# samuelkriegerbonini-dev/AstroBurst

Hardware: AMD Instinct MI355X
Metric: MPix/s sigma-clipped stack+stretch, 64x4096x4096 f32 (higher is better)
Workload: dtype f32

## Files before the change

### astroburst_amd/csrc/tile_stream.hpp

```cpp
#pragma once
#include <hip/hip_runtime.h>

#include <cstdint>

#include "ab_common.hpp"
#include "tile_bucket.hpp"

namespace ts {

using tb::dev_key;
using tb::wave_scan_incl;
using tb::wave_sort64;
using tb::Window;

constexpr int kThreads = 256;
constexpr int kWaves = kThreads / 64;
constexpr int kBuckets = 4096;
constexpr int kTop = kBuckets - 1;
constexpr int kPer = kBuckets / kThreads;
constexpr int kHotCap = 3072;
constexpr int kTabCap = 384;
constexpr int kSelCap = 1024;
constexpr int kMaxZones = 16;
constexpr int kRing = 2;
constexpr int kRingPlan = 3;
constexpr int kEdgePlan = 12;
#ifndef TS_PER_SIGMA
#define TS_PER_SIGMA 480.0f
#endif
constexpr float kPerSigma = TS_PER_SIGMA;
constexpr unsigned int kNone = 0xffffffffu;

enum Decline {
    D_NONE = 0, D_ZONES, D_HOT_OVERFLOW, D_MED_CATCHALL, D_MED_COLD, D_MED_BIG, D_DEV_BM, D_DEV_NOFIRST, D_DEV_SHAPE, D_DEV_COLD,
    D_DEV_BIG, D_DEV_COUNT, D_DEV_PROOF, D_EDGE_COLD, D_EDGE_CATCHALL, D_SAMPLE
};

struct alignas(16) Shared {
    unsigned int prefix[kBuckets + kThreads];
    float list[kHotCap + kThreads];
    union {
        unsigned char lut[kBuckets];
        unsigned int tmp[kSelCap];
    };
    unsigned int zcur[kMaxZones + kThreads];
    uint32_t tab_first[kTabCap], tab_last[kTabCap];
    unsigned int part[4 * kWaves];
    unsigned int zone_at[kMaxZones + 1];
    int zone_lo[kMaxZones], zone_hi[kMaxZones];
    int zone_tab[kMaxZones];
    int nzones;
    int decline;
    unsigned int ncand;
#ifdef AB_TILE_TIMING
    long long t_phase[16];
    long long t_mark;
#endif
};

#ifdef AB_TILE_TIMING
#define TS_MARK(sh, i)                             \
    do {                                           \
        if (threadIdx.x == 0) {                    \
            const long long now_ = clock64();      \
            (sh).t_phase[i] += now_ - (sh).t_mark; \
            (sh).t_mark = now_;                    \
        }                                          \
    } while (0)
#else
#define TS_MARK(sh, i) \
    do {               \
    } while (0)
#endif

__device__ __forceinline__ uint32_t ord_of(float x) {
    const uint32_t b = __float_as_uint(x);
    return b ^ ((b >> 31) ? 0xffffffffu : 0x80000000u);
}
__device__ __forceinline__ float from_ord(uint32_t u) { return __uint_as_float(u ^ ((u >> 31) ? 0x80000000u : 0xffffffffu)); }

struct Geo {
    float scale, off;
    float r_min, r_max;
    ab_pixel_xf xf;
    double range;
    __device__ __forceinline__ int bucket(float v) const { return (int)__builtin_amdgcn_fmed3f(__builtin_fmaf(v, scale, off), 0.0f, (float)kTop); }
    __device__ __forceinline__ bool is_cand(float v) const { return v >= r_min && v <= r_max; }
    __device__ __forceinline__ uint32_t norm_key(float raw) const { return __float_as_uint(ab_px(xf, raw)); }
    __device__ __forceinline__ float unnorm(float x) const { return xf.on ? (float)((double)x * range + xf.lo) : x; }
    __device__ __forceinline__ int bucket_at_norm(float x) const { return bucket(unnorm(x)); }
    __device__ __forceinline__ bool first_raw(int b, float *out) const {
        uint32_t u = ord_of(((float)b - off) / scale);
        int guard = 0;
        while (bucket(from_ord(u)) >= b && ++guard < 64) --u;
        while (bucket(from_ord(u)) < b && ++guard < 128) ++u;
        *out = from_ord(u);
        return guard < 128 && bucket(from_ord(u)) >= b && bucket(from_ord(u - 1u)) < b;
    }
    __device__ __forceinline__ bool first_norm(int b, uint32_t *key) const {
        if (b <= 0) {
            *key = 0x33d6bf96u;
            return true;
        }
        float r;
        if (!first_raw(b, &r)) return false;
        *key = norm_key(r < r_min ? r_min : r);
        return true;
    }
    __device__ __forceinline__ bool last_norm(int b, uint32_t *key) const {
        if (b >= kTop) {
            *key = norm_key(r_max);
            return true;
        }
        float r;
        if (!first_raw(b + 1, &r)) return false;
        r = from_ord(ord_of(r) - 1u);
        *key = norm_key(r < r_min ? r_min : r);
        return true;
    }
};

__device__ __forceinline__ void scan_prefix(Shared &sh) {
    const int t = threadIdx.x, b0 = t * kPer, w = t >> 6, lane = t & 63;
    unsigned int v[kPer];
#pragma unroll
    for (int j = 0; j < kPer; j += 4) {
        const uint4 q = *reinterpret_cast<const uint4 *>(&sh.prefix[b0 + j]);
        v[j] = q.x;
        v[j + 1] = q.y;
        v[j + 2] = q.z;
        v[j + 3] = q.w;
    }
#pragma unroll
    for (int j = 1; j < kPer; ++j) v[j] += v[j - 1];
    const unsigned int tot = v[kPer - 1], incl = wave_scan_incl(tot);
    if (lane == 63) sh.part[w] = incl;
    __syncthreads();
    unsigned int before = incl - tot;
#pragma unroll
    for (int i = 0; i < kWaves; ++i) before += i < w ? sh.part[i] : 0u;
#pragma unroll
    for (int j = 0; j < kPer; j += 4) {
        uint4 q;
        q.x = v[j] + before;
        q.y = v[j + 1] + before;
        q.z = v[j + 2] + before;
        q.w = v[j + 3] + before;
        *reinterpret_cast<uint4 *>(&sh.prefix[b0 + j]) = q;
    }
    __syncthreads();
}

__device__ __forceinline__ void wave_sync() { __builtin_amdgcn_fence(__ATOMIC_ACQ_REL, "wavefront"); }
__device__ __forceinline__ int first_lane(unsigned long long m) { return (int)__builtin_ctzll(m); }
__device__ __forceinline__ unsigned int lanes_below(unsigned long long m) {
    return __builtin_amdgcn_mbcnt_hi((unsigned int)(m >> 32), __builtin_amdgcn_mbcnt_lo((unsigned int)m, 0u));
}
__device__ __forceinline__ unsigned int below(const Shared &sh, int b) { return b <= 0 ? 0u : sh.prefix[b - 1]; }

__device__ __forceinline__ int wfind_rank(const Shared &sh, unsigned int g) {
    const int lane = threadIdx.x & 63;
    const unsigned long long m1 = __builtin_amdgcn_ballot_w64(g < sh.prefix[64 * lane + 63]);
    const int L = m1 ? first_lane(m1) : 63;
    const unsigned long long m2 = __builtin_amdgcn_ballot_w64(g < sh.prefix[64 * L + lane]);
    return 64 * L + (m2 ? first_lane(m2) : 63);
}

__device__ __forceinline__ unsigned int wprefix(const Shared &sh, const Window &w, int b) {
    const unsigned int p = below(sh, b);
    const unsigned int q = p < w.c_lo ? w.c_lo : (p > w.c_le_hi ? w.c_le_hi : p);
    return q - w.c_lo;
}

struct ZReg {
    int lo, hi, tab;
    unsigned int at, end;
    int n;
    __device__ __forceinline__ void load(const Shared &sh) {
        const int lane = threadIdx.x & 63;
        n = sh.nzones;
        const bool have = lane < n;
        lo = have ? sh.zone_lo[lane] : 0;
        hi = have ? sh.zone_hi[lane] : -1;
        tab = have ? sh.zone_tab[lane] : -1;
        at = have ? sh.zone_at[lane] : 0u;
        end = have ? sh.zone_at[lane + 1] : 0u;
    }
    __device__ __forceinline__ int zone_of(int b) const {
        const unsigned long long m = __builtin_amdgcn_ballot_w64(b >= lo && b <= hi);
        return m ? first_lane(m) : -1;
    }
    __device__ __forceinline__ int lo_of(int z) const { return __builtin_amdgcn_readlane(lo, z); }
    __device__ __forceinline__ int hi_of(int z) const { return __builtin_amdgcn_readlane(hi, z); }
    __device__ __forceinline__ unsigned int at_of(int z) const { return (unsigned int)__builtin_amdgcn_readlane((int)at, z); }
    __device__ __forceinline__ unsigned int end_of(int z) const { return (unsigned int)__builtin_amdgcn_readlane((int)end, z); }
    __device__ __forceinline__ int tab_index(int b) const {
        const unsigned long long m = __builtin_amdgcn_ballot_w64(tab >= 0 && b >= lo - 1 && b <= hi + 1);
        if (!m) return -1;
        const int z = first_lane(m);
        return __builtin_amdgcn_readlane(tab, z) + (b - __builtin_amdgcn_readlane(lo, z) + 1);
    }
};
__device__ __forceinline__ bool tfirst(const Shared &sh, const ZReg &zr, const Geo &g, int b, uint32_t *key) {
    const int i = zr.tab_index(b);
    if (i < 0) return g.first_norm(b, key);
    *key = sh.tab_first[i];
    return *key != 0u;
}
__device__ __forceinline__ bool tlast(const Shared &sh, const ZReg &zr, const Geo &g, int b, uint32_t *key) {
    const int i = zr.tab_index(b);
    if (i < 0) return g.last_norm(b, key);
    *key = sh.tab_last[i];
    return *key != 0u;
}

struct DevGeo {
    float mf;
    float delta;
    int bm;
};
__device__ __forceinline__ void ring_of(const Geo &g, const DevGeo &d, float t, int *bl, int *br) {
    const int l = g.bucket_at_norm(d.mf - t), r = g.bucket_at_norm(d.mf + t);
    *bl = l < d.bm ? l : d.bm;
    *br = r > d.bm ? r : d.bm;
}
__device__ __forceinline__ bool make_devgeo(const Shared &sh, const ZReg &zr, const Geo &g, double median, DevGeo *d) {
    d->mf = (float)median;
    int b = g.bucket_at_norm(d->mf), guard = 0;
    uint32_t k;
    auto first_le = [&](int bb, bool *le) {
        if (!tfirst(sh, zr, g, bb, &k)) return false;
        *le = (double)__uint_as_float(k) <= median;
        return true;
    };
    bool le;
    while (b > 0) {
        if (!first_le(b, &le)) return false;
        if (le || ++guard > 8) break;
        --b;
    }
    while (b < kTop) {
        if (!first_le(b + 1, &le)) return false;
        if (!le || ++guard > 16) break;
        ++b;
    }
    d->bm = b;
    if (b <= 0 || b >= kTop || guard > 16) return false;
    uint32_t k0, k1;
    if (!tfirst(sh, zr, g, b, &k0) || !tfirst(sh, zr, g, b + 1, &k1)) return false;
    d->delta = __uint_as_float(k1) - __uint_as_float(k0);
    return d->delta > 0.0f;
}

__device__ __forceinline__ unsigned int wmad_first(const Shared &sh, const Geo &g, const Window &w, const DevGeo &d, unsigned int need, unsigned int guess) {
    const int lane = threadIdx.x & 63;
    auto reaches = [&](unsigned int i) {
        int bl, br;
        ring_of(g, d, (float)(i + 1u) * d.delta, &bl, &br);
        return wprefix(sh, w, br + 1) - wprefix(sh, w, bl) >= need;
    };
    if (guess != kNone) {
        const unsigned int gi = guess < 3900u ? guess : 3900u, i_lo = gi > 96u ? gi - 96u : 0u;
#pragma unroll 1
        for (int j = 0; j < 4; ++j) {
            const unsigned long long m = __builtin_amdgcn_ballot_w64(reaches(i_lo + 64u * j + lane));
            if (m) {
                const unsigned int first = i_lo + 64u * j + (unsigned int)first_lane(m);
                if (first > i_lo || i_lo == 0u) return first;
                break;
            }
        }
    }
#pragma unroll 1
    for (int j = 0; j < kBuckets / 64; ++j) {
        const unsigned long long m = __builtin_amdgcn_ballot_w64(reaches(64u * j + lane));
        if (m) return 64u * j + (unsigned int)first_lane(m);
    }
    return kNone;
}

__device__ __forceinline__ int plan_zones(Shared &sh, const Geo &g, unsigned int cnt, float mad_guess, unsigned int (&first_guess)[3]) {
    int nz = 0;
    auto add = [&](int lo, int hi) {
        lo = lo < 1 ? 1 : lo;
        hi = hi > kTop - 1 ? kTop - 1 : hi;
        if (lo <= hi && nz < kMaxZones) {
            if ((threadIdx.x & 63) == 0) {
                sh.zone_lo[nz] = lo;
                sh.zone_hi[nz] = hi;
            }
            ++nz;
        }
    };
    Window w;
    w.lo = 1;
    w.hi = 0x7f7fffffu;
    w.c_lo = 0;
    w.c_le_hi = cnt;
    w.n = cnt;
    first_guess[0] = first_guess[1] = first_guess[2] = kNone;
#pragma unroll 1
    for (int it = 0; it < 3; ++it) {
        if (w.n < 3) break;
        const unsigned int mid = w.n / 2, g_hi = w.c_lo + mid, g_lo = w.n % 2 == 0 ? g_hi - 1 : g_hi;
        const int b_hi = wfind_rank(sh, g_hi), b_lo = g_lo == g_hi ? b_hi : wfind_rank(sh, g_lo);
        add(b_lo - 1, b_hi + 1);
        if (b_hi <= 0 || b_hi >= kTop) break;
        uint32_t k0, k1;
        if (!g.first_norm(b_hi, &k0) || !g.first_norm(b_hi + 1, &k1)) break;
        const unsigned int ex = below(sh, b_hi), in_b = sh.prefix[b_hi] - ex;
        const float frac = ((float)(g_hi - ex) + 0.5f) / (float)(in_b ? in_b : 1u);
        const float v0 = __uint_as_float(k0), v1 = __uint_as_float(k1);
        const double med = (double)(v0 + frac * (v1 - v0));
        DevGeo d;
        d.mf = (float)med;
        d.bm = b_hi;
        d.delta = v1 - v0;
        if (!(d.delta > 0.0f)) break;
        unsigned int guess = kNone;
        if (it == 0) {
            if (mad_guess > 0.0f) {
                const float gi = mad_guess / d.delta;
                guess = gi < 3900.0f ? (unsigned int)gi : 3900u;
            }
        } else {
            guess = first_guess[it - 1];
        }
        const unsigned int first = wmad_first(sh, g, w, d, mid + 1u, guess);
        if (first == kNone) break;
        first_guess[it] = first;
        {
            int bLo, bRo, bLi = d.bm, bRi = d.bm;
            ring_of(g, d, (float)(first + 1u + kRing + kRingPlan) * d.delta, &bLo, &bRo);
            if (first + 1u > (unsigned int)(kRing + kRingPlan)) ring_of(g, d, (float)(first + 1u - kRing - kRingPlan) * d.delta, &bLi, &bRi);
            if (bLi + 1 >= bRi) {
                add(bLo, bRo);
            } else {
                add(bLo, bLi);
                add(bRi, bRo);
            }
        }
        if (it == 2) break;
        const double mad = (double)(((float)first + 0.5f) * d.delta);
        const double sig = fmax(mad * 1.4826, 1e-30);
        const float lo = (float)(med - 3.0 * sig), hi = (float)(med + 3.0 * sig);
        if (!(lo <= hi)) break;
        const float e = (float)kEdgePlan * d.delta;
        int bl = 0, bh = kTop;
        if (lo > 0.0f) {
            add(g.bucket_at_norm(lo - e), g.bucket_at_norm(lo + e));
            bl = g.bucket_at_norm(lo);
        }
        if (hi < 3.0e38f) {
            add(g.bucket_at_norm(hi - e), g.bucket_at_norm(hi + e));
            bh = g.bucket_at_norm(hi);
        }
        unsigned int c_lo = lo > 0.0f ? below(sh, bl) + (sh.prefix[bl] - below(sh, bl)) / 2u : 0u;
        unsigned int c_hi = hi < 3.0e38f ? sh.prefix[bh] - (sh.prefix[bh] - below(sh, bh)) / 2u : cnt;
        c_lo = c_lo > w.c_lo ? c_lo : w.c_lo;
        c_hi = c_hi < w.c_le_hi ? c_hi : w.c_le_hi;
        if (c_hi <= c_lo) break;
        w.c_lo = c_lo;
        w.c_le_hi = c_hi;
        w.n = c_hi - c_lo;
    }
    return nz;
}

__device__ __forceinline__ bool build_zones(Shared &sh, const Geo &g, int nz) {
    const int lane = threadIdx.x & 63;
    wave_sync();
    uint32_t key = lane < nz ? ((uint32_t)sh.zone_lo[lane] << 16) | (uint32_t)sh.zone_hi[lane] : kNone;
    key = wave_sort64(key);
    int m = 0, cur_lo = 0, cur_hi = -2;
    int my_lo = 0, my_hi = -1;
    for (int i = 0; i < nz; ++i) {
        const uint32_t k = (uint32_t)__builtin_amdgcn_readlane((int)key, i);
        const int lo = (int)(k >> 16), hi = (int)(k & 0xffffu);
        if (m > 0 && lo <= cur_hi + 1) {
            cur_hi = hi > cur_hi ? hi : cur_hi;
        } else {
            if (m > 0 && lane == m - 1) {
                my_lo = cur_lo;
                my_hi = cur_hi;
            }
            cur_lo = lo;
            cur_hi = hi;
            ++m;
        }
    }
    if (m > 0 && lane == m - 1) {
        my_lo = cur_lo;
        my_hi = cur_hi;
    }
    const unsigned int size = lane < m ? sh.prefix[my_hi] - below(sh, my_lo) : 0u;
    const unsigned int tlen = lane < m ? (unsigned int)(my_hi - my_lo + 3) : 0u;
    const unsigned int at = wave_scan_incl(size) - size, tat = wave_scan_incl(tlen) - tlen;
    if (lane < m) {
        sh.zone_lo[lane] = my_lo;
        sh.zone_hi[lane] = my_hi;
        sh.zone_at[lane] = at;
        sh.zcur[lane] = at;
        sh.zone_tab[lane] = tat + tlen <= (unsigned int)kTabCap ? (int)tat : -1;
        if (lane == m - 1) sh.zone_at[m] = at + size;
    }
    if (lane == 0) sh.nzones = m;
    wave_sync();
    return m != 0 && sh.zone_at[m] <= (unsigned int)kHotCap;
}
__device__ __forceinline__ void fill_zone_tables(Shared &sh, const Geo &g) {
    const int t = threadIdx.x, m = sh.nzones;
    for (int z = 0; z < m; ++z) {
        const int lo = sh.zone_lo[z], hi = sh.zone_hi[z], tb0 = sh.zone_tab[z];
        for (int b = lo + t; b <= hi; b += kThreads) sh.lut[b] = (unsigned char)(z + 1);
        if (tb0 >= 0)
            for (int b = lo - 1 + t; b <= hi + 1; b += kThreads) {
                uint32_t kf = 0u, kl = 0u;
                if (!g.first_norm(b, &kf)) kf = 0u;
                if (!g.last_norm(b, &kl)) kl = 0u;
                sh.tab_first[tb0 + (b - lo + 1)] = kf;
                sh.tab_last[tb0 + (b - lo + 1)] = kl;
            }
    }
}

__device__ __forceinline__ void wselect2(Shared &sh, unsigned int n, unsigned int r_lo, unsigned int r_hi, uint32_t *k_lo, uint32_t *k_hi) {
    constexpr int kMine = kSelCap / 64;
    const int lane = threadIdx.x & 63;
    unsigned int *const hist = &sh.prefix[kBuckets];
    wave_sync();
    if (n <= 64u) {
        const uint32_t sorted = wave_sort64((unsigned int)lane < n ? sh.tmp[lane] : kNone);
        *k_lo = (uint32_t)__builtin_amdgcn_readlane((int)sorted, (int)r_lo);
        *k_hi = (uint32_t)__builtin_amdgcn_readlane((int)sorted, (int)r_hi);
        return;
    }
    uint32_t mine[kMine];
    const uint32_t k0 = sh.tmp[0];
    uint32_t diff = 0;
#pragma unroll
    for (int q = 0; q < kMine; ++q) {
        const unsigned int i = (unsigned int)(q * 64 + lane);
        mine[q] = i < n ? sh.tmp[i] : k0;
        diff |= mine[q] ^ k0;
    }
#pragma unroll
    for (int off = 32; off >= 1; off >>= 1) diff |= (uint32_t)__shfl_xor((int)diff, off, 64);
    int top = 24;
    while (top > 0 && (diff >> top) == 0) top -= 8;
    uint32_t mask = top == 24 ? 0u : (0xffffffffu << (top + 8));
    uint32_t prefix = k0 & mask;
    unsigned int rank = r_hi;
    for (int shift = top; shift >= 0; shift -= 8) {
        *reinterpret_cast<uint4 *>(&hist[4 * lane]) = make_uint4(0u, 0u, 0u, 0u);
        wave_sync();
#pragma unroll
        for (int q = 0; q < kMine; ++q)
            if ((unsigned int)(q * 64) < n) {
                if ((unsigned int)(q * 64 + lane) < n && (mine[q] & mask) == prefix) atomicAdd(&hist[(mine[q] >> shift) & 255u], 1u);
            }
        wave_sync();
        const uint4 c = *reinterpret_cast<const uint4 *>(&hist[4 * lane]);
        const unsigned int own = c.x + c.y + c.z + c.w;
        const unsigned int incl = wave_scan_incl(own);
        const unsigned int excl = incl - own;
        const bool owner = rank >= excl && rank < incl;
        uint32_t digit = 0;
        unsigned int bel = 0;
        if (owner) {
            const unsigned int r = rank - excl;
            if (r < c.x) {
                digit = 4 * lane;
                bel = excl;
            } else if (r < c.x + c.y) {
                digit = 4 * lane + 1;
                bel = excl + c.x;
            } else if (r < c.x + c.y + c.z) {
                digit = 4 * lane + 2;
                bel = excl + c.x + c.y;
            } else {
                digit = 4 * lane + 3;
                bel = excl + c.x + c.y + c.z;
            }
        }
        const unsigned long long om = __builtin_amdgcn_ballot_w64(owner);
        const int ol = om ? first_lane(om) : 0;
        digit = (uint32_t)__builtin_amdgcn_readlane((int)digit, ol);
        bel = (unsigned int)__builtin_amdgcn_readlane((int)bel, ol);
        rank -= bel;
        prefix |= digit << shift;
        mask |= 255u << shift;
    }
    *k_hi = prefix;
    *k_lo = prefix;
    if (r_lo != r_hi && rank == 0) {
        uint32_t best = 0;
#pragma unroll
        for (int q = 0; q < kMine; ++q)
            if ((unsigned int)(q * 64 + lane) < n && mine[q] < prefix) best = best > mine[q] ? best : mine[q];
        *k_lo = tb::wave_max(best);
    }
}

template <class KeyOf>
__device__ __forceinline__ unsigned int gather_keys(Shared &sh, unsigned int from, unsigned int to, uint32_t k_from, uint32_t k_to, unsigned int at,
                                                    KeyOf key_of) {
    const int lane = threadIdx.x & 63;
    const uint32_t *const list = reinterpret_cast<const uint32_t *>(sh.list);
#pragma unroll 1
    for (unsigned int i0 = from; i0 < to; i0 += 256) {
        uint32_t key[4];
#pragma unroll
        for (int j = 0; j < 4; ++j) {
            const unsigned int i = i0 + 64u * j + lane;
            const uint32_t k = i < to ? list[i] : 0u;
            key[j] = (k >= k_from && k <= k_to) ? key_of(k) : kNone;
        }
#pragma unroll
        for (int j = 0; j < 4; ++j) {
            const unsigned long long m = __builtin_amdgcn_ballot_w64(key[j] != kNone);
            const unsigned int pos = at + lanes_below(m);
            if (key[j] != kNone && pos < (unsigned int)kSelCap) sh.tmp[pos] = key[j];
            at += (unsigned int)__builtin_popcountll(m);
        }
        if (at > (unsigned int)kSelCap) return kNone;
    }
    return at;
}

struct Rounds {
    Shared &sh;
    const Geo &g;
    ZReg zr;
    __device__ __forceinline__ bool fail(int why) {
        sh.decline = why;
        return false;
    }
    __device__ __forceinline__ bool key_range(int ba, int bb, uint32_t *k_from, uint32_t *k_to) {
        uint32_t prev, next;
        if (!tfirst(sh, zr, g, ba, k_from) || !tlast(sh, zr, g, bb, k_to) || !tlast(sh, zr, g, ba - 1, &prev) || !tfirst(sh, zr, g, bb + 1, &next)) return false;
        if (prev >= *k_from && sh.prefix[ba - 1] != below(sh, ba - 1)) return false;
        if (next <= *k_to && sh.prefix[bb + 1] != sh.prefix[bb]) return false;
        return true;
    }
    __device__ __forceinline__ bool select_values(unsigned int g_lo, unsigned int g_hi, uint32_t *k_lo, uint32_t *k_hi) {
        const int b_hi = wfind_rank(sh, g_hi), b_lo = g_lo == g_hi ? b_hi : wfind_rank(sh, g_lo);
        if (b_lo <= 0 || b_hi >= kTop) return fail(D_MED_CATCHALL);
        const int z_lo = zr.zone_of(b_lo), z_hi = zr.zone_of(b_hi);
        if (z_lo < 0 || z_hi < 0) return fail(D_MED_COLD);
        auto same = [](uint32_t k) { return k; };
        uint32_t kf, kt;
        if (!key_range(b_lo, b_lo, &kf, &kt)) return fail(D_MED_COLD);
        unsigned int n = gather_keys(sh, zr.at_of(z_lo), zr.end_of(z_lo), kf, kt, 0u, same);
        if (n != kNone && b_hi != b_lo) {
            if (!key_range(b_hi, b_hi, &kf, &kt)) return fail(D_MED_COLD);
            n = gather_keys(sh, zr.at_of(z_hi), zr.end_of(z_hi), kf, kt, n, same);
        }
        if (n == kNone) return fail(D_MED_BIG);
        const unsigned int ex = below(sh, b_lo);
        if (n != sh.prefix[b_hi] - ex) return fail(D_MED_COLD);
        TS_MARK(sh, 8);
        wselect2(sh, n, g_lo - ex, g_hi - ex, k_lo, k_hi);
        TS_MARK(sh, 9);
        return true;
    }
    __device__ __forceinline__ bool select_devs(const Window &w, double median, unsigned int r_lo, unsigned int r_hi, unsigned int guess, uint32_t *d_lo,
                                                uint32_t *d_hi) {
        DevGeo d;
        if (!make_devgeo(sh, zr, g, median, &d)) return fail(D_DEV_BM);
        TS_MARK(sh, 10);
        const unsigned int first = wmad_first(sh, g, w, d, r_hi + 1u, guess);
        TS_MARK(sh, 11);
        if (first == kNone) return fail(D_DEV_NOFIRST);
        int bLo, bRo, bLi = 0, bRi = 0;
        ring_of(g, d, (float)(first + 1u + kRing) * d.delta, &bLo, &bRo);
        const bool has_inner_t = first + 1u > (unsigned int)kRing;
        if (has_inner_t) ring_of(g, d, (float)(first + 1u - kRing) * d.delta, &bLi, &bRi);
        const bool has_inner = has_inner_t && bLi + 1 <= bRi - 1;
        const unsigned int c_in = has_inner ? wprefix(sh, w, bRi) - wprefix(sh, w, bLi + 1) : 0u;
        const unsigned int n_cand = wprefix(sh, w, bRo + 1) - wprefix(sh, w, bLo) - c_in;
        if (!(bLo > 0 && bRo < kTop && c_in <= r_lo && c_in + n_cand >= r_hi + 1u && n_cand <= (unsigned int)kSelCap)) return fail(D_DEV_SHAPE);
        auto key_of = [&](uint32_t k) { return (k >= w.lo && k <= w.hi) ? dev_key(k, median) : kNone; };
        unsigned int n;
        uint32_t kf, kt;
        if (has_inner) {
            const int zl = zr.zone_of(bLo), zq = zr.zone_of(bRi);
            if (zl < 0 || zq < 0 || bLi > zr.hi_of(zl) || bRo > zr.hi_of(zq)) return fail(D_DEV_COLD);
            if (!key_range(bLo, bLi, &kf, &kt)) return fail(D_DEV_COLD);
            n = gather_keys(sh, zr.at_of(zl), zr.end_of(zl), kf, kt, 0u, key_of);
            if (n != kNone) {
                if (!key_range(bRi, bRo, &kf, &kt)) return fail(D_DEV_COLD);
                n = gather_keys(sh, zr.at_of(zq), zr.end_of(zq), kf, kt, n, key_of);
            }
        } else {
            const int z = zr.zone_of(bLo);
            if (z < 0 || bRo > zr.hi_of(z)) return fail(D_DEV_COLD);
            if (!key_range(bLo, bRo, &kf, &kt)) return fail(D_DEV_COLD);
            n = gather_keys(sh, zr.at_of(z), zr.end_of(z), kf, kt, 0u, key_of);
        }
        if (n == kNone) return fail(D_DEV_BIG);
        if (n != n_cand) return fail(D_DEV_COUNT);
        TS_MARK(sh, 12);
        uint32_t sel_lo, sel_hi;
        wselect2(sh, n, r_lo - c_in, r_hi - c_in, &sel_lo, &sel_hi);
        TS_MARK(sh, 13);
        uint32_t t_in = 0, t_out = kNone;
        if (has_inner) {
            uint32_t ka, kb;
            if (!tfirst(sh, zr, g, bLi + 1, &ka) || !tlast(sh, zr, g, bRi - 1, &kb)) return fail(D_DEV_PROOF);
            ka = ka > w.lo ? ka : w.lo;
            kb = kb < w.hi ? kb : w.hi;
            if (ka <= kb) {
                const uint32_t da = dev_key(ka, median), db = dev_key(kb, median);
                t_in = da > db ? da : db;
            }
        }
        if (wprefix(sh, w, bLo) > 0u) {
            uint32_t k;
            if (!tlast(sh, zr, g, bLo - 1, &k) || !((double)__uint_as_float(k) <= median)) return fail(D_DEV_PROOF);
            t_out = dev_key(k, median);
        }
        if (wprefix(sh, w, kBuckets) - wprefix(sh, w, bRo + 1) > 0u) {
            uint32_t k;
            if (!tfirst(sh, zr, g, bRo + 1, &k) || !((double)__uint_as_float(k) >= median)) return fail(D_DEV_PROOF);
            const uint32_t dd = dev_key(k, median);
            t_out = t_out < dd ? t_out : dd;
        }
        TS_MARK(sh, 14);
        if (!(t_in <= sel_lo && sel_hi <= t_out)) return fail(D_DEV_PROOF);
        *d_lo = sel_lo;
        *d_hi = sel_hi;
        return true;
    }
    template <bool HI>
    __device__ __forceinline__ bool count_edge(uint32_t bound, unsigned int *out) {
        const int lane = threadIdx.x & 63;
        int b = g.bucket_at_norm(__uint_as_float(bound)), guard = 0;
        auto reaches = [&](int bb, bool *r) {
            uint32_t k;
            if (!tlast(sh, zr, g, bb, &k)) return false;
            *r = HI ? k > bound : k >= bound;
            return true;
        };
        bool r;
        while (b > 0) {
            if (!reaches(b - 1, &r)) return fail(D_EDGE_COLD);
            if (!r || ++guard > 8) break;
            --b;
        }
        while (b < kTop) {
            if (!reaches(b, &r)) return fail(D_EDGE_COLD);
            if (r || ++guard > 16) break;
            ++b;
        }
        if (guard > 16) return fail(D_EDGE_COLD);
        const unsigned int bel = below(sh, b), in_b = sh.prefix[b] - bel;
        if (in_b == 0) {
            *out = bel;
            return true;
        }
        if (b <= 0 || b >= kTop) {
            uint32_t kf, kl;
            if (!tfirst(sh, zr, g, b, &kf) || !tlast(sh, zr, g, b, &kl)) return fail(D_EDGE_CATCHALL);
            if (HI ? kl <= bound : kl < bound) {
                *out = bel + in_b;
                return true;
            }
            if (HI ? kf > bound : kf >= bound) {
                *out = bel;
                return true;
            }
            return fail(D_EDGE_CATCHALL);
        }
        const int z = zr.zone_of(b);
        uint32_t kf, kt;
        if (z < 0 || !key_range(b, b, &kf, &kt)) return fail(D_EDGE_COLD);
        const uint32_t *const list = reinterpret_cast<const uint32_t *>(sh.list);
        unsigned int c = 0, seen = 0;
        const unsigned int to = zr.end_of(z);
        for (unsigned int i0 = zr.at_of(z); i0 < to; i0 += 256) {
#pragma unroll
            for (int j = 0; j < 4; ++j) {
                const unsigned int i = i0 + 64u * j + lane;
                const uint32_t k = i < to ? list[i] : 0u;
                const bool mine = k >= kf && k <= kt;
                seen += mine ? 1u : 0u;
                c += (mine && (HI ? k <= bound : k < bound)) ? 1u : 0u;
            }
        }
        seen = tb::wave_sum(seen);
        c = tb::wave_sum(c);
        if (seen != in_b) return fail(D_EDGE_COLD);
        *out = bel + c;
        return true;
    }

    __device__ __forceinline__ bool run(unsigned int cnt, const unsigned int (&first_guess)[3], double *median_out, double *sigma_out) {
        constexpr double kMadToSigma = 1.4826;
        zr.load(sh);
        Window w;
        w.lo = 1;
        w.hi = 0x7f7fffffu;
        w.c_lo = 0;
        w.c_le_hi = cnt;
        w.n = cnt;
        double median = 0.0, sigma = 1.0;
#pragma unroll 1
        for (int it = 0; it < 3; ++it) {
            if (it < 2 && w.n < 3) continue;
            if (w.n == 0) {
                median = 0.0;
                sigma = 1.0;
                break;
            }
            const unsigned int mid = w.n / 2;
            uint32_t ka, kb;
            if (!select_values(w.c_lo + (w.n % 2 == 0 ? mid - 1 : mid), w.c_lo + mid, &ka, &kb)) return false;
            median = w.n % 2 == 0 ? ((double)__uint_as_float(ka) + (double)__uint_as_float(kb)) / 2.0 : (double)__uint_as_float(kb);
            uint32_t da, db;
            if (!select_devs(w, median, w.n % 2 == 0 ? mid - 1 : mid, mid, first_guess[it], &da, &db)) return false;
            const float mad_f32 = w.n % 2 == 0 ? (__uint_as_float(da) + __uint_as_float(db)) / 2.0f : __uint_as_float(db);
            const double sig = fmax((double)mad_f32 * kMadToSigma, 1e-30);
            if (it == 2) {
                sigma = sig;
                break;
            }
            const float lo = (float)(median - 3.0 * sig), hi = (float)(median + 3.0 * sig);
            if (!(lo <= hi)) {
                w.n = 0;
                w.c_lo = w.c_le_hi = 0;
                w.lo = 1;
                w.hi = 0;
                continue;
            }
            const uint32_t klo = lo > 0.0f ? __float_as_uint(lo) : 1u;
            const uint32_t khi = hi > 0.0f ? (__float_as_uint(hi) > 0x7f7fffffu ? 0x7f7fffffu : __float_as_uint(hi)) : 0u;
            const bool new_lo = klo > w.lo, new_hi = khi < w.hi;
            w.lo = new_lo ? klo : w.lo;
            w.hi = new_hi ? khi : w.hi;
            if (w.lo > w.hi) {
                w.n = 0;
                w.c_lo = w.c_le_hi = 0;
                continue;
            }
            TS_MARK(sh, 6);
            if (new_lo && w.lo > 0x33d6bf96u && !count_edge<false>(w.lo, &w.c_lo)) return false;
            if (new_hi && !count_edge<true>(w.hi, &w.c_le_hi)) return false;
            w.n = w.c_le_hi - w.c_lo;
            TS_MARK(sh, 15);
        }
        *median_out = median;
        *sigma_out = sigma;
        return true;
    }
};

struct TileRect {
    const float *img;
    int64_t ld;
    int y0, y1, x0, x1;
    bool vec;
};
struct __attribute__((packed, aligned(4))) F4u {
    float x, y, z, w;
};
__device__ __forceinline__ float4 load4u(const float *p) {
    const F4u t = *reinterpret_cast<const F4u *>(p);
    return make_float4(t.x, t.y, t.z, t.w);
}
__device__ __forceinline__ bool whole_tile(const TileRect &r) { return r.vec && r.y1 - r.y0 == 256 && r.x1 - r.x0 == 256; }
template <class F>
__device__ __forceinline__ void stream_whole_tile_batches(const TileRect &r, F f) {
    constexpr int U = 4, kRounds = 64 / (2 * U);
    const int t = threadIdx.x, lane = t & 63, wv = t >> 6;
    const float *p = r.img + (int64_t)(r.y0 + wv) * r.ld + r.x0 + 4 * lane;
    const int64_t step = (int64_t)kWaves * r.ld;
    float4 A[U], B[U];
    auto load = [&](float4(&X)[U]) {
#pragma unroll
        for (int u = 0; u < U; ++u) X[u] = load4u(p + u * step);
        p += U * step;
    };
    unsigned int at = (unsigned int)(wv * 256 + 4 * lane);
    auto eat = [&](const float4(&X)[U]) {
        float v[4 * U];
#pragma unroll
        for (int u = 0; u < U; ++u) {
            v[4 * u + 0] = X[u].x;
            v[4 * u + 1] = X[u].y;
            v[4 * u + 2] = X[u].z;
            v[4 * u + 3] = X[u].w;
        }
        f(v, at);
        at += (unsigned int)(U * kWaves * 256);
    };
    load(A);
#pragma unroll 1
    for (int it = 0; it < kRounds; ++it) {
        load(B);
        eat(A);
        if (it + 1 < kRounds) load(A);
        eat(B);
    }
}
template <class F>
__device__ __forceinline__ void stream_tile(const TileRect &r, F f) {
    const int t = threadIdx.x;
    if (whole_tile(r)) {
        constexpr int U = 4, kRounds = 64 / (2 * U);
        const int lane = t & 63, wv = t >> 6;
        const float *p = r.img + (int64_t)(r.y0 + wv) * r.ld + r.x0 + 4 * lane;
        const int64_t step = (int64_t)kWaves * r.ld;
        float4 A[U], B[U];
        auto load = [&](float4(&X)[U]) {
#pragma unroll
            for (int u = 0; u < U; ++u) X[u] = load4u(p + u * step);
            p += U * step;
        };
        auto eat = [&](const float4(&X)[U]) {
#pragma unroll
            for (int u = 0; u < U; ++u) {
                f(X[u].x);
                f(X[u].y);
                f(X[u].z);
                f(X[u].w);
            }
        };
        load(A);
#pragma unroll 1
        for (int it = 0; it < kRounds; ++it) {
            load(B);
            eat(A);
            if (it + 1 < kRounds) load(A);
            eat(B);
        }
    } else if (r.vec) {
        constexpr int U = 8;
        const int lane = t & 63, wv = t >> 6, c = r.x0 + 4 * lane;
        const bool col_ok = c < r.x1;
        const float *p = r.img + c;
#pragma unroll 1
        for (int r0 = r.y0 + wv; r0 < r.y1; r0 += kWaves * U) {
            float4 raw[U];
#pragma unroll
            for (int u = 0; u < U; ++u) {
                const int row = r0 + kWaves * u;
                raw[u] = (col_ok && row < r.y1) ? load4u(p + (int64_t)row * r.ld)
                                                : make_float4(__builtin_nanf(""), __builtin_nanf(""), __builtin_nanf(""), __builtin_nanf(""));
            }
#pragma unroll
            for (int u = 0; u < U; ++u) {
                f(raw[u].x);
                f(raw[u].y);
                f(raw[u].z);
                f(raw[u].w);
            }
        }
    } else {
        constexpr int U = 16;
        const int c = r.x0 + t;
        const bool col_ok = c < r.x1;
        const float *p = r.img + c;
#pragma unroll 1
        for (int r0 = r.y0; r0 < r.y1; r0 += U) {
            float raw[U];
#pragma unroll
            for (int u = 0; u < U; ++u) raw[u] = (col_ok && r0 + u < r.y1) ? p[(int64_t)(r0 + u) * r.ld] : __builtin_nanf("");
#pragma unroll
            for (int u = 0; u < U; ++u) f(raw[u]);
        }
    }
}

struct TileResult {
    double median, sigma;
    int valid;
    int declined;
};

__device__ __forceinline__ void candidate_range(const ab_pixel_xf &xf, float *r_min, float *r_max) {
    if (!xf.on) {
        *r_min = __uint_as_float(0x33d6bf96u);
        *r_max = 3.4028234663852886e38f;
        return;
    }
    *r_max = __builtin_inff();
    uint32_t lo = ord_of(-__builtin_inff()), hi = ord_of(__builtin_inff());
    while (hi - lo > 1u) {
        const uint32_t mid = lo + ((hi - lo) >> 1);
        if (ab_px(xf, from_ord(mid)) > 1e-7f)
            hi = mid;
        else
            lo = mid;
    }
    *r_min = from_ord(hi);
}

__device__ __forceinline__ bool zoom_from_sample(Shared &sh, const TileRect &r, const ab_pixel_xf &xf, Geo *g, float *mad_guess) {
    const int t = threadIdx.x, lane = t & 63, wv = t >> 6;
    const int h = r.y1 - r.y0, wd = r.x1 - r.x0;
    g->xf = xf;
    g->range = xf.on ? 1.0 / xf.inv : 1.0;
    candidate_range(xf, &g->r_min, &g->r_max);
    const int sr = r.y0 + (int)(((unsigned int)t * (unsigned int)h) >> 8), sc = r.x0 + (int)(((unsigned int)(t * 67 + 13) % 256u * (unsigned int)wd) >> 8);
    const float sv = r.img[(int64_t)sr * r.ld + sc];
    const uint32_t sorted = wave_sort64(g->is_cand(sv) ? ord_of(sv) : 0u);
    const int nz = __builtin_popcountll(__builtin_amdgcn_ballot_w64(sorted == 0u)), nv = 64 - nz;
    const uint32_t q1 = (uint32_t)__shfl((int)sorted, nz + nv / 4 < 64 ? nz + nv / 4 : 63, 64);
    const uint32_t q2 = (uint32_t)__shfl((int)sorted, nz + nv / 2 < 64 ? nz + nv / 2 : 63, 64);
    const uint32_t q3 = (uint32_t)__shfl((int)sorted, nz + (3 * nv) / 4 < 64 ? nz + (3 * nv) / 4 : 63, 64);
    if (lane == 0) {
        sh.part[4 * wv + 0] = q1;
        sh.part[4 * wv + 1] = q2;
        sh.part[4 * wv + 2] = q3;
        sh.part[4 * wv + 3] = nv >= 8 ? 1u : 0u;
    }
    __syncthreads();
    float s1 = 0.0f, s2 = 0.0f, s3 = 0.0f, sn = 0.0f;
#pragma unroll
    for (int i = 0; i < kWaves; ++i) {
        const bool ok = sh.part[4 * i + 3] != 0u;
        s1 += ok ? from_ord(sh.part[4 * i + 0]) : 0.0f;
        s2 += ok ? from_ord(sh.part[4 * i + 1]) : 0.0f;
        s3 += ok ? from_ord(sh.part[4 * i + 2]) : 0.0f;
        sn += ok ? 1.0f : 0.0f;
    }
    __syncthreads();
    if (!(sn > 0.0f)) return false;
    const float Q1 = s1 / sn, Q2 = s2 / sn, Q3 = s3 / sn;
    const float sig = (Q3 - Q1) * (1.0f / 1.349f);
    const float wb = sig / kPerSigma;
    g->scale = 1.0f / wb;
    const float vlo = Q2 - (float)((kBuckets - 2) / 2) * wb;
    g->off = 1.0f - vlo * g->scale;
    *mad_guess = 0.6745f * sig * (float)(xf.on ? xf.inv : 1.0);
    return sig > 0.0f && __builtin_isfinite(g->scale) && __builtin_isfinite(g->off) && g->scale > 0.0f;
}

struct CandSink {
    uint2 *ent = nullptr;
    unsigned int *cnt = nullptr;
    float *cut = nullptr;
    unsigned int cap = 0;
};
#ifndef TS_CAND_SIGMAS
#define TS_CAND_SIGMAS 2.5f
#endif
constexpr float kCandSigmas = TS_CAND_SIGMAS;

__device__ __forceinline__ int rounds_wave() {
#ifdef TS_ROUNDS_WAVE0
    return 0;
#else
    return (int)(blockIdx.x & 3u);
#endif
}

__device__ __forceinline__ TileResult tile_stats(Shared &sh, const TileRect &r, const ab_pixel_xf &xf, const CandSink cs = CandSink()) {
    const int t = threadIdx.x;
    TileResult res = {0.0, 1.0, 0, 0};
    if (cs.cut && t == 0) {
        *cs.cut = __builtin_nanf("");
        *cs.cnt = 0u;
    }
#ifdef AB_TILE_TIMING
    if (t == 0) {
        for (int i = 0; i < 16; ++i) sh.t_phase[i] = 0;
        sh.t_mark = clock64();
    }
#endif
    if (t == 0) {
        sh.decline = D_NONE;
        sh.nzones = 0;
        sh.ncand = 0u;
    }
#pragma unroll
    for (int i = 0; i < kPer; i += 4) *reinterpret_cast<uint4 *>(&sh.prefix[t * kPer + i]) = make_uint4(0u, 0u, 0u, 0u);
    *reinterpret_cast<uint4 *>(&sh.lut[16 * t]) = make_uint4(0u, 0u, 0u, 0u);
    Geo g;
    float mad_guess;
    if (!zoom_from_sample(sh, r, xf, &g, &mad_guess)) {
        res.declined = D_SAMPLE;
        return res;
    }
    TS_MARK(sh, 0);
    stream_tile(r, [&](float v) { atomicAdd(&sh.prefix[g.is_cand(v) ? g.bucket(v) : kBuckets + t], 1u); });
    __syncthreads();
    TS_MARK(sh, 1);
    scan_prefix(sh);
    const unsigned int cnt = sh.prefix[kTop];
    TS_MARK(sh, 2);
    if (cnt < 8) return res;
    res.valid = 1;
    unsigned int first_guess[3] = {kNone, kNone, kNone};
    const int rw = rounds_wave();
    if ((t >> 6) == rw) {
        const int nz = plan_zones(sh, g, cnt, mad_guess, first_guess);
        TS_MARK(sh, 3);
        if (!build_zones(sh, g, nz)) sh.decline = sh.nzones == 0 ? D_ZONES : D_HOT_OVERFLOW;
    }
    __syncthreads();
    if (sh.decline) {
        res.declined = sh.decline;
        return res;
    }
    fill_zone_tables(sh, g);
    __syncthreads();
    TS_MARK(sh, 4);
    const int cb = (kBuckets - 2) / 2 + 1 + (int)(kCandSigmas * kPerSigma);
    float cut_raw = 0.0f;
    const bool emit = cs.ent != nullptr && cb > 1 && cb < kTop && whole_tile(r) && g.first_raw(cb, &cut_raw);
    if (whole_tile(r)) {
        stream_whole_tile_batches(r, [&](const float(&v)[16], unsigned int pos0) {
            int b[16];
            unsigned int z[16], at[16];
#pragma unroll
            for (int i = 0; i < 16; ++i) b[i] = g.bucket(v[i]);
#pragma unroll
            for (int i = 0; i < 16; ++i) z[i] = sh.lut[b[i]];
#pragma unroll
            for (int i = 0; i < 16; ++i) z[i] = g.is_cand(v[i]) ? z[i] : 0u;
#pragma unroll
            for (int i = 0; i < 16; ++i) at[i] = atomicAdd(&sh.zcur[z[i] ? z[i] - 1u : (unsigned int)(kMaxZones + t)], 1u);
#pragma unroll
            for (int i = 0; i < 16; ++i) sh.list[(z[i] && at[i] < (unsigned int)kHotCap) ? at[i] : (unsigned int)(kHotCap + t)] = v[i];
            if (emit) {
                unsigned int hit = 0;
#pragma unroll
                for (int i = 0; i < 16; ++i) hit |= (b[i] >= cb && v[i] <= g.r_max) ? 1u << i : 0u;
                while (hit) {
                    const int i = __builtin_ctz(hit);
                    hit &= hit - 1u;
                    const unsigned int ca = atomicAdd(&sh.ncand, 1u);
                    float vi = v[0];
#pragma unroll
                    for (int k = 1; k < 16; ++k) vi = i == k ? v[k] : vi;
                    if (ca < cs.cap) cs.ent[ca] = make_uint2(pos0 + (unsigned int)((i >> 2) * (kWaves * 256) + (i & 3)), __float_as_uint(vi));
                }
            }
        });
    } else {
        stream_tile(r, [&](float v) {
            unsigned int z = sh.lut[g.bucket(v)];
            z = g.is_cand(v) ? z : 0u;
            const unsigned int at = atomicAdd(&sh.zcur[z ? z - 1u : (unsigned int)(kMaxZones + t)], 1u);
            sh.list[(z && at < (unsigned int)kHotCap) ? at : (unsigned int)(kHotCap + t)] = v;
        });
    }
    __syncthreads();
    if (emit && t == 0) {
        *cs.cnt = sh.ncand;
        *cs.cut = cut_raw;
    }
    {
        const unsigned int n = sh.zone_at[sh.nzones];
        for (unsigned int i = t; i < n; i += kThreads) sh.list[i] = __uint_as_float(g.norm_key(sh.list[i]));
    }
    __syncthreads();
    TS_MARK(sh, 5);
#ifdef AB_TILE_TIMING
    if (t == 0) sh.t_phase[7] = sh.zone_at[sh.nzones] * 1000 + sh.nzones;
#endif
    if ((t >> 6) != rw) return res;
    Rounds rounds = {sh, g, ZReg()};
    if (!rounds.run(cnt, first_guess, &res.median, &res.sigma)) res.declined = sh.decline ? sh.decline : 1;
    TS_MARK(sh, 6);
    return res;
}

}
```

Baseline: 110,300.

## Bucket-sort hot list by bucket so selections read contiguous slices

Replaces the in-place key normalization pass with order_hot_list, which counting-sorts the hot-zone values by bucket using per-bucket atomic cursors in shared memory. Later median, deviation and edge-count steps can then read exact contiguous slices instead of scanning whole zones and filtering by key range. A single-zone median selection can read keys directly from the list without a gather. This adds several block barriers and atomics per tile, plus new declines when the hot bucket count exceeds capacity or the per-bucket counts fail verification.

```diff
diff --git a/astroburst_amd/csrc/tile_stream.hpp b/astroburst_amd/csrc/tile_stream.hpp
--- a/astroburst_amd/csrc/tile_stream.hpp
+++ b/astroburst_amd/csrc/tile_stream.hpp
@@ -30,10 +30,12 @@
 #endif
 constexpr float kPerSigma = TS_PER_SIGMA;
 constexpr unsigned int kNone = 0xffffffffu;
+constexpr int kPhases = 17;
+static_assert(kSelCap == 4 * kThreads && kHotCap % kThreads == 0 && kMaxZones <= 4 * kWaves, "order_hot_list: cursors cleared four per thread, the list read in whole rows of threads");
 
 enum Decline {
     D_NONE = 0, D_ZONES, D_HOT_OVERFLOW, D_MED_CATCHALL, D_MED_COLD, D_MED_BIG, D_DEV_BM, D_DEV_NOFIRST, D_DEV_SHAPE, D_DEV_COLD,
-    D_DEV_BIG, D_DEV_COUNT, D_DEV_PROOF, D_EDGE_COLD, D_EDGE_CATCHALL, D_SAMPLE
+    D_DEV_BIG, D_DEV_COUNT, D_DEV_PROOF, D_EDGE_COLD, D_EDGE_CATCHALL, D_SAMPLE, D_HOT_BUCKETS, D_HOT_ORDER
 };
 
 struct alignas(16) Shared {
@@ -45,7 +47,10 @@
     };
     unsigned int zcur[kMaxZones + kThreads];
     uint32_t tab_first[kTabCap], tab_last[kTabCap];
-    unsigned int part[4 * kWaves];
+    union {
+        unsigned int part[4 * kWaves];
+        unsigned int zone_slot[kMaxZones];
+    };
     unsigned int zone_at[kMaxZones + 1];
     int zone_lo[kMaxZones], zone_hi[kMaxZones];
     int zone_tab[kMaxZones];
@@ -53,7 +58,7 @@
     int decline;
     unsigned int ncand;
 #ifdef AB_TILE_TIMING
-    long long t_phase[16];
+    long long t_phase[kPhases];
     long long t_mark;
 #endif
 };
@@ -174,7 +179,7 @@
 
 struct ZReg {
     int lo, hi, tab;
-    unsigned int at, end;
+    unsigned int shift;
     int n;
     __device__ __forceinline__ void load(const Shared &sh) {
         const int lane = threadIdx.x & 63;
@@ -183,8 +188,7 @@
         lo = have ? sh.zone_lo[lane] : 0;
         hi = have ? sh.zone_hi[lane] : -1;
         tab = have ? sh.zone_tab[lane] : -1;
-        at = have ? sh.zone_at[lane] : 0u;
-        end = have ? sh.zone_at[lane + 1] : 0u;
+        shift = have ? sh.zone_at[lane] - below(sh, lo) : 0u;
     }
     __device__ __forceinline__ int zone_of(int b) const {
         const unsigned long long m = __builtin_amdgcn_ballot_w64(b >= lo && b <= hi);
@@ -192,8 +196,7 @@
     }
     __device__ __forceinline__ int lo_of(int z) const { return __builtin_amdgcn_readlane(lo, z); }
     __device__ __forceinline__ int hi_of(int z) const { return __builtin_amdgcn_readlane(hi, z); }
-    __device__ __forceinline__ unsigned int at_of(int z) const { return (unsigned int)__builtin_amdgcn_readlane((int)at, z); }
-    __device__ __forceinline__ unsigned int end_of(int z) const { return (unsigned int)__builtin_amdgcn_readlane((int)end, z); }
+    __device__ __forceinline__ unsigned int shift_of(int z) const { return (unsigned int)__builtin_amdgcn_readlane((int)shift, z); }
     __device__ __forceinline__ int tab_index(int b) const {
         const unsigned long long m = __builtin_amdgcn_ballot_w64(tab >= 0 && b >= lo - 1 && b <= hi + 1);
         if (!m) return -1;
@@ -367,7 +370,7 @@
     return nz;
 }
 
-__device__ __forceinline__ bool build_zones(Shared &sh, const Geo &g, int nz) {
+__device__ __forceinline__ Decline build_zones(Shared &sh, const Geo &g, int nz) {
     const int lane = threadIdx.x & 63;
     wave_sync();
     uint32_t key = lane < nz ? ((uint32_t)sh.zone_lo[lane] << 16) | (uint32_t)sh.zone_hi[lane] : kNone;
@@ -402,11 +405,15 @@
         sh.zone_at[lane] = at;
         sh.zcur[lane] = at;
         sh.zone_tab[lane] = tat + tlen <= (unsigned int)kTabCap ? (int)tat : -1;
+        sh.zone_slot[lane] = tat - 2u * (unsigned int)lane;
         if (lane == m - 1) sh.zone_at[m] = at + size;
     }
     if (lane == 0) sh.nzones = m;
     wave_sync();
-    return m != 0 && sh.zone_at[m] <= (unsigned int)kHotCap;
+    if (m == 0) return D_ZONES;
+    if (sh.zone_at[m] > (unsigned int)kHotCap) return D_HOT_OVERFLOW;
+    const unsigned int hot_buckets = (unsigned int)__builtin_amdgcn_readlane((int)(tat + tlen), m - 1) - 2u * (unsigned int)m;
+    return hot_buckets <= (unsigned int)kSelCap ? D_NONE : D_HOT_BUCKETS;
 }
 __device__ __forceinline__ void fill_zone_tables(Shared &sh, const Geo &g) {
     const int t = threadIdx.x, m = sh.nzones;
@@ -424,24 +431,66 @@
     }
 }
 
-__device__ __forceinline__ void wselect2(Shared &sh, unsigned int n, unsigned int r_lo, unsigned int r_hi, uint32_t *k_lo, uint32_t *k_hi) {
+__device__ __forceinline__ void order_hot_list(Shared &sh, const Geo &g) {
+    constexpr int kMine = kHotCap / kThreads;
+    const int t = threadIdx.x, m = sh.nzones;
+    const unsigned int n = sh.zone_at[m];
+    uint32_t key[kMine];
+    unsigned int slot[kMine], first[kMine];
+#pragma unroll
+    for (int j = 0; j < kMine; ++j) {
+        slot[j] = kNone;
+        if ((unsigned int)(j * kThreads) < n) {
+            const unsigned int i = (unsigned int)(j * kThreads + t);
+            const float v = i < n ? sh.list[i] : 0.0f;
+            const int b = g.bucket(v);
+            const unsigned int z1 = i < n ? sh.lut[b] : 0u;
+            const int z = z1 ? (int)z1 - 1 : 0, lo = sh.zone_lo[z];
+            key[j] = g.norm_key(v);
+            first[j] = sh.zone_at[z] - below(sh, lo) + below(sh, b);
+            if (z1) slot[j] = sh.zone_slot[z] + (unsigned int)(b - lo);
+        }
+    }
+    __syncthreads();
+    *reinterpret_cast<uint4 *>(&sh.tmp[4 * t]) = make_uint4(0u, 0u, 0u, 0u);
+    __syncthreads();
+    unsigned int at[kMine];
+#pragma unroll
+    for (int j = 0; j < kMine; ++j)
+        if (slot[j] != kNone) at[j] = first[j] + atomicAdd(&sh.tmp[slot[j]], 1u);
+#pragma unroll
+    for (int j = 0; j < kMine; ++j)
+        if (slot[j] != kNone && at[j] < n) reinterpret_cast<uint32_t *>(sh.list)[at[j]] = key[j];
+    __syncthreads();
+    bool ok = true;
+    for (int z = 0; z < m; ++z) {
+        const int lo = sh.zone_lo[z], hi = sh.zone_hi[z];
+        const unsigned int s0 = sh.zone_slot[z];
+        for (int b = lo + t; b <= hi; b += kThreads) ok = ok && sh.tmp[s0 + (unsigned int)(b - lo)] == sh.prefix[b] - below(sh, b);
+    }
+    if (!ok) sh.decline = D_HOT_ORDER;
+    __syncthreads();
+}
+
+__device__ __forceinline__ void wselect2(Shared &sh, const uint32_t *keys, unsigned int n, unsigned int r_lo, unsigned int r_hi, uint32_t *k_lo,
+                                         uint32_t *k_hi) {
     constexpr int kMine = kSelCap / 64;
     const int lane = threadIdx.x & 63;
     unsigned int *const hist = &sh.prefix[kBuckets];
     wave_sync();
     if (n <= 64u) {
-        const uint32_t sorted = wave_sort64((unsigned int)lane < n ? sh.tmp[lane] : kNone);
+        const uint32_t sorted = wave_sort64((unsigned int)lane < n ? keys[lane] : kNone);
         *k_lo = (uint32_t)__builtin_amdgcn_readlane((int)sorted, (int)r_lo);
         *k_hi = (uint32_t)__builtin_amdgcn_readlane((int)sorted, (int)r_hi);
         return;
     }
     uint32_t mine[kMine];
-    const uint32_t k0 = sh.tmp[0];
+    const uint32_t k0 = keys[0];
     uint32_t diff = 0;
 #pragma unroll
     for (int q = 0; q < kMine; ++q) {
         const unsigned int i = (unsigned int)(q * 64 + lane);
-        mine[q] = i < n ? sh.tmp[i] : k0;
+        mine[q] = i < n ? keys[i] : k0;
         diff |= mine[q] ^ k0;
     }
 #pragma unroll
@@ -503,8 +552,7 @@
 }
 
 template <class KeyOf>
-__device__ __forceinline__ unsigned int gather_keys(Shared &sh, unsigned int from, unsigned int to, uint32_t k_from, uint32_t k_to, unsigned int at,
-                                                    KeyOf key_of) {
+__device__ __forceinline__ unsigned int gather_keys(Shared &sh, unsigned int from, unsigned int to, unsigned int at, KeyOf key_of) {
     const int lane = threadIdx.x & 63;
     const uint32_t *const list = reinterpret_cast<const uint32_t *>(sh.list);
 #pragma unroll 1
@@ -513,8 +561,7 @@
 #pragma unroll
         for (int j = 0; j < 4; ++j) {
             const unsigned int i = i0 + 64u * j + lane;
-            const uint32_t k = i < to ? list[i] : 0u;
-            key[j] = (k >= k_from && k <= k_to) ? key_of(k) : kNone;
+            key[j] = i < to ? key_of(list[i]) : kNone;
         }
 #pragma unroll
         for (int j = 0; j < 4; ++j) {
@@ -536,31 +583,32 @@
         sh.decline = why;
         return false;
     }
-    __device__ __forceinline__ bool key_range(int ba, int bb, uint32_t *k_from, uint32_t *k_to) {
-        uint32_t prev, next;
-        if (!tfirst(sh, zr, g, ba, k_from) || !tlast(sh, zr, g, bb, k_to) || !tlast(sh, zr, g, ba - 1, &prev) || !tfirst(sh, zr, g, bb + 1, &next)) return false;
-        if (prev >= *k_from && sh.prefix[ba - 1] != below(sh, ba - 1)) return false;
-        if (next <= *k_to && sh.prefix[bb + 1] != sh.prefix[bb]) return false;
-        return true;
+    __device__ __forceinline__ void slice(int z, int ba, int bb, unsigned int *from, unsigned int *to) const {
+        const unsigned int s = zr.shift_of(z);
+        *from = s + below(sh, ba);
+        *to = s + sh.prefix[bb];
     }
     __device__ __forceinline__ bool select_values(unsigned int g_lo, unsigned int g_hi, uint32_t *k_lo, uint32_t *k_hi) {
         const int b_hi = wfind_rank(sh, g_hi), b_lo = g_lo == g_hi ? b_hi : wfind_rank(sh, g_lo);
         if (b_lo <= 0 || b_hi >= kTop) return fail(D_MED_CATCHALL);
         const int z_lo = zr.zone_of(b_lo), z_hi = zr.zone_of(b_hi);
         if (z_lo < 0 || z_hi < 0) return fail(D_MED_COLD);
-        auto same = [](uint32_t k) { return k; };
-        uint32_t kf, kt;
-        if (!key_range(b_lo, b_lo, &kf, &kt)) return fail(D_MED_COLD);
-        unsigned int n = gather_keys(sh, zr.at_of(z_lo), zr.end_of(z_lo), kf, kt, 0u, same);
-        if (n != kNone && b_hi != b_lo) {
-            if (!key_range(b_hi, b_hi, &kf, &kt)) return fail(D_MED_COLD);
-            n = gather_keys(sh, zr.at_of(z_hi), zr.end_of(z_hi), kf, kt, n, same);
-        }
-        if (n == kNone) return fail(D_MED_BIG);
-        const unsigned int ex = below(sh, b_lo);
-        if (n != sh.prefix[b_hi] - ex) return fail(D_MED_COLD);
+        const unsigned int ex = below(sh, b_lo), n = sh.prefix[b_hi] - ex;
+        if (n > (unsigned int)kSelCap) return fail(D_MED_BIG);
+        const uint32_t *keys = sh.tmp;
+        unsigned int from, to;
+        if (z_lo == z_hi) {
+            slice(z_lo, b_lo, b_hi, &from, &to);
+            keys = reinterpret_cast<const uint32_t *>(sh.list) + from;
+        } else {
+            auto same = [](uint32_t k) { return k; };
+            slice(z_lo, b_lo, b_lo, &from, &to);
+            const unsigned int n_lo = gather_keys(sh, from, to, 0u, same);
+            slice(z_hi, b_hi, b_hi, &from, &to);
+            if (n_lo == kNone || gather_keys(sh, from, to, n_lo, same) != n) return fail(D_MED_COLD);
+        }
         TS_MARK(sh, 8);
-        wselect2(sh, n, g_lo - ex, g_hi - ex, k_lo, k_hi);
+        wselect2(sh, keys, n, g_lo - ex, g_hi - ex, k_lo, k_hi);
         TS_MARK(sh, 9);
         return true;
     }
@@ -581,28 +629,27 @@
         const unsigned int n_cand = wprefix(sh, w, bRo + 1) - wprefix(sh, w, bLo) - c_in;
         if (!(bLo > 0 && bRo < kTop && c_in <= r_lo && c_in + n_cand >= r_hi + 1u && n_cand <= (unsigned int)kSelCap)) return fail(D_DEV_SHAPE);
         auto key_of = [&](uint32_t k) { return (k >= w.lo && k <= w.hi) ? dev_key(k, median) : kNone; };
-        unsigned int n;
-        uint32_t kf, kt;
+        unsigned int n, from, to;
         if (has_inner) {
             const int zl = zr.zone_of(bLo), zq = zr.zone_of(bRi);
             if (zl < 0 || zq < 0 || bLi > zr.hi_of(zl) || bRo > zr.hi_of(zq)) return fail(D_DEV_COLD);
-            if (!key_range(bLo, bLi, &kf, &kt)) return fail(D_DEV_COLD);
-            n = gather_keys(sh, zr.at_of(zl), zr.end_of(zl), kf, kt, 0u, key_of);
+            slice(zl, bLo, bLi, &from, &to);
+            n = gather_keys(sh, from, to, 0u, key_of);
             if (n != kNone) {
-                if (!key_range(bRi, bRo, &kf, &kt)) return fail(D_DEV_COLD);
-                n = gather_keys(sh, zr.at_of(zq), zr.end_of(zq), kf, kt, n, key_of);
+                slice(zq, bRi, bRo, &from, &to);
+                n = gather_keys(sh, from, to, n, key_of);
             }
         } else {
             const int z = zr.zone_of(bLo);
             if (z < 0 || bRo > zr.hi_of(z)) return fail(D_DEV_COLD);
-            if (!key_range(bLo, bRo, &kf, &kt)) return fail(D_DEV_COLD);
-            n = gather_keys(sh, zr.at_of(z), zr.end_of(z), kf, kt, 0u, key_of);
+            slice(z, bLo, bRo, &from, &to);
+            n = gather_keys(sh, from, to, 0u, key_of);
         }
         if (n == kNone) return fail(D_DEV_BIG);
         if (n != n_cand) return fail(D_DEV_COUNT);
         TS_MARK(sh, 12);
         uint32_t sel_lo, sel_hi;
-        wselect2(sh, n, r_lo - c_in, r_hi - c_in, &sel_lo, &sel_hi);
+        wselect2(sh, sh.tmp, n, r_lo - c_in, r_hi - c_in, &sel_lo, &sel_hi);
         TS_MARK(sh, 13);
         uint32_t t_in = 0, t_out = kNone;
         if (has_inner) {
@@ -673,24 +720,18 @@
             return fail(D_EDGE_CATCHALL);
         }
         const int z = zr.zone_of(b);
-        uint32_t kf, kt;
-        if (z < 0 || !key_range(b, b, &kf, &kt)) return fail(D_EDGE_COLD);
+        if (z < 0) return fail(D_EDGE_COLD);
         const uint32_t *const list = reinterpret_cast<const uint32_t *>(sh.list);
-        unsigned int c = 0, seen = 0;
-        const unsigned int to = zr.end_of(z);
-        for (unsigned int i0 = zr.at_of(z); i0 < to; i0 += 256) {
+        unsigned int c = 0, from, to;
+        slice(z, b, b, &from, &to);
+        for (unsigned int i0 = from; i0 < to; i0 += 256) {
 #pragma unroll
             for (int j = 0; j < 4; ++j) {
                 const unsigned int i = i0 + 64u * j + lane;
-                const uint32_t k = i < to ? list[i] : 0u;
-                const bool mine = k >= kf && k <= kt;
-                seen += mine ? 1u : 0u;
-                c += (mine && (HI ? k <= bound : k < bound)) ? 1u : 0u;
-            }
-        }
-        seen = tb::wave_sum(seen);
+                c += (i < to && (HI ? list[i] <= bound : list[i] < bound)) ? 1u : 0u;
+            }
+        }
         c = tb::wave_sum(c);
-        if (seen != in_b) return fail(D_EDGE_COLD);
         *out = bel + c;
         return true;
     }
@@ -965,7 +1006,7 @@
     }
 #ifdef AB_TILE_TIMING
     if (t == 0) {
-        for (int i = 0; i < 16; ++i) sh.t_phase[i] = 0;
+        for (int i = 0; i < kPhases; ++i) sh.t_phase[i] = 0;
         sh.t_mark = clock64();
     }
 #endif
@@ -997,7 +1038,8 @@
     if ((t >> 6) == rw) {
         const int nz = plan_zones(sh, g, cnt, mad_guess, first_guess);
         TS_MARK(sh, 3);
-        if (!build_zones(sh, g, nz)) sh.decline = sh.nzones == 0 ? D_ZONES : D_HOT_OVERFLOW;
+        const Decline why = build_zones(sh, g, nz);
+        if (why != D_NONE) sh.decline = why;
     }
     __syncthreads();
     if (sh.decline) {
@@ -1052,16 +1094,17 @@
         *cs.cnt = sh.ncand;
         *cs.cut = cut_raw;
     }
-    {
-        const unsigned int n = sh.zone_at[sh.nzones];
-        for (unsigned int i = t; i < n; i += kThreads) sh.list[i] = __uint_as_float(g.norm_key(sh.list[i]));
-    }
-    __syncthreads();
     TS_MARK(sh, 5);
+    order_hot_list(sh, g);
+    TS_MARK(sh, 16);
 #ifdef AB_TILE_TIMING
     if (t == 0) sh.t_phase[7] = sh.zone_at[sh.nzones] * 1000 + sh.nzones;
 #endif
     if ((t >> 6) != rw) return res;
+    if (sh.decline) {
+        res.declined = sh.decline;
+        return res;
+    }
     Rounds rounds = {sh, g, ZReg()};
     if (!rounds.run(cnt, first_guess, &res.median, &res.sigma)) res.declined = sh.decline ? sh.decline : 1;
     TS_MARK(sh, 6);
```

Measured after the change: 112,100 (median of 2 runs). About the same (+1.6%).
